# microsoft/CoCosNet

Measured on AMD Instinct MI355X. Metric: images/sec fwd+bwd ADE20k 256x256 batch-8/GPU (correspondence hot path), higher is better.
Workload: dtype f32 (K2 products as 3-term f16 hi/lo split on the f16 MFMA, fp32 accumulate); 1 GPU; ADE20k 256x256 batch 8/GPU, 64x64 grid (HW=4096), K=256, Cv=154 (rgb+151 labels), match_kernel 1, PONO_C, T=0.01; precision=f16x3; scope=hotpath: theta/phi 1x1 conv + centre/L2norm + fused corr-softmax-warp fwd+bwd; global_batch=8, parallelism=dp1, grad_payload=path, grad_allreduce_bytes=0

## Files before the change

### cocosnet_amd/csrc/corr_fused_fwd_f16x3.hip

```cpp
#include "common.h"
#include <type_traits>

namespace cocos {

typedef _Float16 f16x8 __attribute__((ext_vector_type(8)));
typedef _Float16 f16x2 __attribute__((ext_vector_type(2)));
typedef unsigned int u32x2 __attribute__((ext_vector_type(2)));

constexpr int SP_BQ = 128;
constexpr int SP_BK = 32;
constexpr int SP_KD = 256;
constexpr int SP_KROW = SP_KD + 8;
constexpr int SP_VROW = 40;
constexpr float kSplitRescaleThr = 6.0f;
constexpr float kPBias = 15.0f - kSplitRescaleThr;

__device__ __forceinline__ f32x16 mfma16h(f16x8 a, f16x8 b, f32x16 c) {
    return __builtin_amdgcn_mfma_f32_32x32x16_f16(a, b, c, 0, 0, 0);
}
__device__ __forceinline__ f16x8 buf_load_h8(__amdgpu_buffer_rsrc_t r, unsigned byte_off) {
    return __builtin_bit_cast(f16x8, __builtin_amdgcn_raw_buffer_load_b128(r, (int)byte_off, 0, 0));
}
__device__ __forceinline__ u32x4 buf_load_u4(__amdgpu_buffer_rsrc_t r, unsigned byte_off) {
    return __builtin_amdgcn_raw_buffer_load_b128(r, (int)byte_off, 0, 0);
// ... 14 lines not shown
    split_pair_rtz_lo_scaled(a, b, h, l);
    hi = __builtin_bit_cast(f16x2, h);
    lo = __builtin_bit_cast(f16x2, l);
}

constexpr int kStreamAux = 2;
#ifdef COCOS_DEBUG_TIMING
__device__ long long g_phase_fwd_h[8];
#define FPH_T(var) const long long var = __builtin_readcyclecounter()
#define FPH_ADD(i, a, b) do { if (blockIdx.x == 0 && threadIdx.x == 0) g_phase_fwd_h[i] += (b) - (a); } while (0)
#else
#define FPH_T(var) do {} while (0)
#define FPH_ADD(i, a, b) do {} while (0)
#endif

template <int CVB, bool STORE_S, bool RAGGED, bool VLO0, bool RAWM = false, int KST = SP_KD / 16>
__device__ __forceinline__ void corr_fwd_f16x3_body(
    const _Float16* __restrict__ qh, const _Float16* __restrict__ ql, const _Float16* __restrict__ kh,
    const _Float16* __restrict__ kl, const _Float16* __restrict__ vh, const _Float16* __restrict__ vl,
    float* __restrict__ out, float* __restrict__ lse, float* __restrict__ lg, const float* __restrict__ v_scale,
    const unsigned* __restrict__ v_lo_mask, int B, int Nq, int Nk, int Cv, float scale_log2 ,
    size_t k_bstride ,
    size_t v_bstride ,
    float* __restrict__ rowstat = nullptr ,
    float* __restrict__ mtile = nullptr ) {
    static_assert(KST >= 1 && KST <= SP_KD / 16 && (RAWM || KST == SP_KD / 16), "KST < 16 belongs to the magnitude-free flavour");
    constexpr int CVP = CVB * 32;
    constexpr int KPLANE = SP_BK * SP_KROW;
    constexpr int VPLANE = CVP * SP_VROW;
    extern __shared__ __attribute__((aligned(16))) unsigned char smem_raw[];
    _Float16* const kt = reinterpret_cast<_Float16*>(smem_raw);
    _Float16* const vt = kt + 2 * 2 * KPLANE;

    const int tid = threadIdx.x;
    const int lane = tid & 63, wave = tid >> 6;
    const int h = lane >> 5, c = lane & 31;

    const int nqb = (Nq + SP_BQ - 1) / SP_BQ;
    const int vb = xcd_remap(blockIdx.x, gridDim.x);
    const int b = vb / nqb, qb = vb % nqb;
    const int i_lane = qb * SP_BQ + wave * 32 + c;
// ... 123 lines not shown
    __syncthreads();

    constexpr int RA = 4, NS = SP_KD / 16;
    f16x8 ah[RA], al[RA];
    auto prefetch_k = [&](int buf) {
        const _Float16* kb = kt + buf * 2 * KPLANE + c * SP_KROW + h * 8;
#pragma unroll
        for (int s = 0; s < (RA - 1 < KST ? RA - 1 : KST); ++s) {
            ah[s] = *reinterpret_cast<const f16x8*>(kb + s * 16);
            al[s] = *reinterpret_cast<const f16x8*>(kb + KPLANE + s * 16);
        }
    };
    prefetch_k(0);

    const std::integral_constant<bool, VLO0> vlo0_tag{};
    for (int t = 0; t < ntiles; ++t) {
        const int j0 = t * SP_BK, buf = t & 1;
        const bool ragged = RAGGED && (j0 + SP_BK > Nk);
        _Float16* const kw = kt + (buf ^ 1) * 2 * KPLANE;
        _Float16* const vw = vt + (buf ^ 1) * 3 * VPLANE;
        const int jn = j0 + 2 * SP_BK;
        auto piece = [&](int i, auto vlo0_piece_tag) __attribute__((always_inline)) {
            constexpr bool PLO0 = decltype(vlo0_piece_tag)::value;
            if (!RAGGED) {
                const int jc = min(jn, Nk - SP_BK);
                if (i < 8) {
                    const int pl_ = i & 1, u = i >> 1;
                    *reinterpret_cast<u32x4*>(kw + pl_ * KPLANE + k_lds[u]) = kst[pl_][u];
                    kst[pl_][u] = buf_load_u4s(pl_ ? kl_rs : kh_rs, k_voff[u], (unsigned)jc * (unsigned)(SP_KD * 2));
                } else if (i - 8 < 2 * CVB) {
                    const int pl_ = (i - 8) & 1, u = (i - 8) >> 1;
                    if (PLO0 && pl_ == 1 && u >= 1) return;
                    const bool ones = pl_ == 0 && u == CVB - 1 && ones_thread;
                    *reinterpret_cast<u32x2*>(vw + pl_ * VPLANE + v_lds[u]) = ones ? kOnes2 : vst[pl_][u];
                    if (pl_ == 0) *reinterpret_cast<u32x2*>(vw + 2 * VPLANE + v_lds[u]) = ones ? kOnesS2 : unshift2(vst[0][u]);
                    vst[pl_][u] = buf_load_u2s(pl_ ? vl_rs : vh_rs, v_voff[u], (unsigned)jc * 2u);
                }
                return;
            }
            if (i < 8) {
                const int pl_ = i & 1, u = i >> 1;
                const int g = u * 256 + tid, key = g >> 5, cc = g & 31;
                *reinterpret_cast<u32x4*>(kw + pl_ * KPLANE + key * SP_KROW + cc * 8) = kst[pl_][u];
                kst[pl_][u] = buf_load_u4(pl_ ? kl_rs : kh_rs, (unsigned)((jn + key) * SP_KD + cc * 8) * 2u);
            } else if (i - 8 < 2 * CVB) {
                const int pl_ = (i - 8) & 1, u = (i - 8) >> 1;
                if (PLO0 && pl_ == 1 && u >= 1) return;
                const int g = u * 256 + tid, row = g >> 3, kq = g & 7;
                const int slot = 16 * (kq >> 2) + 8 * (kq & 1) + 4 * ((kq >> 1) & 1);
                const bool ones = pl_ == 0 && u == CVB - 1 && ones_thread;
                *reinterpret_cast<u32x2*>(vw + pl_ * VPLANE + row * SP_VROW + slot) = ones ? kOnes2 : vst[pl_][u];
                if (pl_ == 0) *reinterpret_cast<u32x2*>(vw + 2 * VPLANE + row * SP_VROW + slot) = ones ? kOnesS2 : unshift2(vst[0][u]);
                unsigned off = (unsigned)(row * Nk + jn + 4 * kq) * 2u;
                if (row >= Cv || jn + 4 * kq >= Nk) off = kBufOob;
                vst[pl_][u] = buf_load_u2(pl_ ? vl_rs : vh_rs, off);
            }
        };

        FPH_T(tp0);
        constexpr bool QK1 = !RAWM;
        f32x16 sa, sb, sc;
#pragma unroll
        for (int r = 0; r < 16; ++r) { sa[r] = RAWM ? -m_run : 0.f; sb[r] = RAWM ? -m_lo : 0.f; sc[r] = 0.f; }
        {
            const _Float16* kb = kt + buf * 2 * KPLANE + c * SP_KROW + h * 8;
#pragma unroll
            for (int s = 0; s < NS; ++s) {
                const int cur = s % RA;
                const bool live = s < KST;
                if (live) sa = mfma16h(ah[cur], qhr[s], sa);
                if (s + RA - 1 < KST) ah[(s + RA - 1) % RA] = *reinterpret_cast<const f16x8*>(kb + (s + RA - 1) * 16);
                __builtin_amdgcn_sched_barrier(0);
                if (live) { if (QK1) sa = mfma16h(ah[cur], qlr[s], sa); else sb = mfma16h(ah[cur], qlr[s], sb); }
                if (s + RA - 1 < KST) al[(s + RA - 1) % RA] = *reinterpret_cast<const f16x8*>(kb + KPLANE + (s + RA - 1) * 16);
                __builtin_amdgcn_sched_barrier(0);
                if (live) { if (QK1) sa = mfma16h(al[cur], qhr[s], sa); else sc = mfma16h(al[cur], qhr[s], sc); }
                if ((s & 1) == 0) piece(s >> 1, std::false_type{});
                __builtin_amdgcn_sched_barrier(0);
            }
        }
        FPH_T(tp1);
        __syncthreads();
        FPH_T(tp2);
        constexpr int NSV = 2 * CVB;
        f16x8 a_h[RA], a_l[RA], a_s[RA];
        const _Float16* vbase = vt + buf * 3 * VPLANE + c * SP_VROW + h * 8;
#pragma unroll
        for (int i = 0; i < RA - 1 && i < NSV; ++i) {
            a_h[i] = *reinterpret_cast<const f16x8*>(vbase + (i % CVB) * 32 * SP_VROW + (i / CVB) * 16);
            a_l[i] = *reinterpret_cast<const f16x8*>(vbase + VPLANE + (i % CVB) * 32 * SP_VROW + (i / CVB) * 16);
            a_s[i] = *reinterpret_cast<const f16x8*>(vbase + 2 * VPLANE + (i % CVB) * 32 * SP_VROW + (i / CVB) * 16);
        }
        f32x16 s0;
#pragma unroll
        for (int r = 0; r < 16; ++r) s0[r] = QK1 ? sa[r] : (sa[r] + sb[r]) + sc[r];
        if (ragged) {
#pragma unroll
            for (int r = 0; r < 16; ++r)
                if (j0 + acc_row_base(r) + 4 * h >= Nk) s0[r] = -INFINITY;
        }
        float tmax = s0[0];
#pragma unroll
        for (int r = 1; r < 16; ++r) tmax = fmaxf(tmax, s0[r]);
        tmax = fmaxf(tmax, swap_half(tmax));
        if (!RAWM) tmax *= scale_log2;
        if (RAWM ? (t == 0 || __any(tmax > thr_raw)) : __any(tmax > m_run + kSplitRescaleThr)) {
            float alpha;
            if (RAWM) {
                const float delta = t == 0 ? tmax : fmaxf(tmax, 0.f);
                alpha = t == 0 ? 1.0f : fast_exp2(-delta * scale_log2);
                const float u = m_lo + delta, ub = u - m_lo;
                const float e1 = (m_lo - (u - ub)) + (delta - ub);
                const float hs = m_run + u, hb = hs - m_run;
                const float e2 = (m_run - (hs - hb)) + (u - hb);
                m_run = hs;
                m_lo = e2 + e1;
#pragma unroll
                for (int r = 0; r < 16; ++r) s0[r] -= delta;
            } else {
                const float m_new = fmaxf(m_run, tmax);
                alpha = fast_exp2(m_run - m_new);
                m_run = m_new;
            }
#pragma unroll
            for (int cb = 0; cb < CVB; ++cb) asm volatile("" : "+a"(o[cb]));
#pragma unroll
            for (int cb = 0; cb < CVB; ++cb)
#pragma unroll
                for (int r = 0; r < 16; ++r) o[cb][r] *= alpha;
#pragma unroll
            for (int cb = 0; cb < CVB; ++cb) asm volatile("" : "+a"(o[cb]));
        }
        if (STORE_S) {
            const unsigned soff = (unsigned)(t * nqblk) * 4096u;
            if (RAWM && mtile && h == 0 && i_lane < Nq) {
                mtile[(((size_t)b * ntiles + t) * 2 + 0) * Nq + i_lane] = m_run;
                mtile[(((size_t)b * ntiles + t) * 2 + 1) * Nq + i_lane] = m_lo;
            }
#pragma unroll
            for (int k = 0; k < 4; ++k)
                __builtin_amdgcn_raw_buffer_store_b128(
                    __builtin_bit_cast(u32x4, f32x4{s0[4 * k], s0[4 * k + 1], s0[4 * k + 2], s0[4 * k + 3]}), lg_rs,
                    (int)lg_lane_off, (int)(soff + (unsigned)k * 1024u), kStreamAux);
        }
        float p[16];
        const float nmb = RAWM ? kPBias : kPBias - m_run;
#pragma unroll
        for (int r = 0; r < 16; ++r) p[r] = fast_exp2(__builtin_fmaf(s0[r], scale_log2, nmb));

        FPH_T(tp3);
        f16x8 ph[2], pl[2];
#pragma unroll
        for (int tt = 0; tt < 2; ++tt)
#pragma unroll
            for (int j = 0; j < 8; j += 2) {
                f16x2 a, bq;
                split_pair(p[8 * tt + j], p[8 * tt + j + 1], a, bq);
                ph[tt][j] = a[0]; ph[tt][j + 1] = a[1];
                pl[tt][j] = bq[0]; pl[tt][j + 1] = bq[1];
            }

        FPH_T(tp4);
        {
#pragma unroll
            for (int i = 0; i < NSV; ++i) {
                const int tt = i / CVB, cb = i % CVB, cur = i % RA, n = i + RA - 1;
                if (n < NSV) {
                    a_h[n % RA] = *reinterpret_cast<const f16x8*>(vbase + (n % CVB) * 32 * SP_VROW + (n / CVB) * 16);
                    a_s[n % RA] = *reinterpret_cast<const f16x8*>(vbase + 2 * VPLANE + (n % CVB) * 32 * SP_VROW + (n / CVB) * 16);
                    if (!VLO0 || (n % CVB) == 0)
                        a_l[n % RA] = *reinterpret_cast<const f16x8*>(vbase + VPLANE + (n % CVB) * 32 * SP_VROW + (n / CVB) * 16);
                }
                o[cb] = mfma16h(a_h[cur], ph[tt], o[cb]);
                o[cb] = mfma16h(a_s[cur], pl[tt], o[cb]);
                if (!VLO0 || cb == 0) o[cb] = mfma16h(a_l[cur], ph[tt], o[cb]);
                piece(8 + i, vlo0_tag);
                if (i == NSV - 1) prefetch_k(buf ^ 1);
                __builtin_amdgcn_sched_barrier(0);
            }
        }
#pragma unroll
        for (int cb = 0; cb < CVB; ++cb) asm volatile("" : "+a"(o[cb]));
        FPH_T(tp5);
        FPH_ADD(0, tp0, tp1); FPH_ADD(1, tp1, tp2); FPH_ADD(2, tp2, tp3); FPH_ADD(3, tp3, tp4);
        FPH_ADD(4, tp4, tp5);
    }

    const float l_own = o[CVB - 1][15];
    const float l_other = swap_half(l_own);
    const float l_tot = h ? l_own : l_other;
    const float inv_l = (v_scale ? 1.0f / *v_scale : 1.0f) / l_tot;
    if (RAWM && rowstat && i_lane < Nq && h == 0) {
        rowstat[((size_t)b * 3 + 0) * Nq + i_lane] = m_run;
        rowstat[((size_t)b * 3 + 1) * Nq + i_lane] = m_lo;
        rowstat[((size_t)b * 3 + 2) * Nq + i_lane] = log2f(l_tot) - kPBias;
    }
    if (RAWM) m_run = (m_run + m_lo) * scale_log2;
    if (i_lane < Nq) {
        float* out_b = out + (size_t)b * Cv * Nq;
#pragma unroll
        for (int cb = 0; cb < CVB; ++cb)
#pragma unroll
            for (int r = 0; r < 16; ++r) {
                const int ch = cb * 32 + acc_row_base(r) + 4 * h;
                if (ch < Cv) out_b[(size_t)ch * Nq + i_lane] = o[cb][r] * inv_l;
            }
        if (h == 0) lse[(size_t)b * Nq + i_lane] = (m_run + log2f(l_tot) - kPBias) * kLn2;
    }
}

template <int CVB, bool STORE_S, bool RAGGED, bool DUAL>
__global__ __launch_bounds__(256, 1) void corr_fwd_f16x3_kernel(
    const _Float16* __restrict__ qh, const _Float16* __restrict__ ql, const _Float16* __restrict__ kh,
    const _Float16* __restrict__ kl, const _Float16* __restrict__ vh, const _Float16* __restrict__ vl,
    float* __restrict__ out, float* __restrict__ lse, float* __restrict__ lg, const float* __restrict__ v_scale,
    const unsigned* __restrict__ v_lo_mask, int B, int Nq, int Nk, int Cv, float scale_log2,
    const float* __restrict__ q_scale_dev, const float* __restrict__ k_scale_dev, float* __restrict__ rowstat,
    float* __restrict__ mtile, int ksteps, size_t k_bstride, size_t v_bstride) {
    if (q_scale_dev) scale_log2 = scale_log2 / (*q_scale_dev * *k_scale_dev);
    if constexpr (DUAL) {
        if ((__builtin_amdgcn_readfirstlane(*v_lo_mask) & ~1u) == 0u)
            corr_fwd_f16x3_body<CVB, STORE_S, RAGGED, true>(qh, ql, kh, kl, vh, vl, out, lse, lg, v_scale, v_lo_mask, B, Nq, Nk, Cv, scale_log2, k_bstride, v_bstride);
        else
            corr_fwd_f16x3_body<CVB, STORE_S, RAGGED, false>(qh, ql, kh, kl, vh, vl, out, lse, lg, v_scale, v_lo_mask, B, Nq, Nk, Cv, scale_log2, k_bstride, v_bstride);
    } else {
        if (q_scale_dev) {
#define COCOS_RAWM_BODY(KST_) corr_fwd_f16x3_body<CVB, STORE_S, RAGGED, false, true, KST_>(qh, ql, kh, kl, vh, vl, out, lse, lg, v_scale, \
                                                                                           v_lo_mask, B, Nq, Nk, Cv, scale_log2, k_bstride, v_bstride, rowstat, mtile)
            if constexpr (RAGGED) {
                COCOS_RAWM_BODY(SP_KD / 16);
            } else {
                if (ksteps <= 2) COCOS_RAWM_BODY(2);
                else if (ksteps <= 4) COCOS_RAWM_BODY(4);
                else if (ksteps <= 8) COCOS_RAWM_BODY(8);
                else COCOS_RAWM_BODY(SP_KD / 16);
            }
#undef COCOS_RAWM_BODY
        } else
            corr_fwd_f16x3_body<CVB, STORE_S, RAGGED, false>(qh, ql, kh, kl, vh, vl, out, lse, lg, v_scale, v_lo_mask, B, Nq, Nk, Cv, scale_log2, k_bstride, v_bstride);
    }
}

template <int CVB, bool STORE_S, bool RAGGED, bool VLO0>
static int launch_f16x3_k(const _Float16* qh, const _Float16* ql, const _Float16* kh, const _Float16* kl,
                          const _Float16* vh, const _Float16* vl, float* out, float* lse, float* lg,
                          const float* v_scale, const unsigned* v_lo_mask, int B, int Nq, int Nk, int Cv, float scale_log2,
                          const float* qsd, const float* ksd, float* rowstat, float* mtile, int ksteps, size_t k_bstride, size_t v_bstride,
                          hipStream_t stream) {
    auto kern = corr_fwd_f16x3_kernel<CVB, STORE_S, RAGGED, VLO0>;
    const size_t smem = (size_t)2 * (2 * SP_BK * SP_KROW + 3 * CVB * 32 * SP_VROW) * sizeof(_Float16);
    COCOS_HIP_CHECK(hipFuncSetAttribute(reinterpret_cast<const void*>(kern),
                                        hipFuncAttributeMaxDynamicSharedMemorySize, (int)smem));
    const int nqb = (Nq + SP_BQ - 1) / SP_BQ;
    hipLaunchKernelGGL(kern, dim3(B * nqb), dim3(256), smem, stream, qh, ql, kh, kl, vh, vl, out, lse, lg, v_scale,
                       v_lo_mask, B, Nq, Nk, Cv, scale_log2, qsd, ksd, rowstat, mtile, ksteps, k_bstride, v_bstride);
    COCOS_HIP_CHECK(hipGetLastError());
    return COCOS_OK;
}

}

#ifdef COCOS_DEBUG_TIMING
extern "C" int cocos_debug_read_timing_fwd_f16x3(long long* host8, int reset) {
    using namespace cocos;
    COCOS_HIP_CHECK(hipDeviceSynchronize());
    COCOS_HIP_CHECK(hipMemcpyFromSymbol(host8, HIP_SYMBOL(g_phase_fwd_h), 8 * sizeof(long long)));
    if (reset) {
        long long z[8] = {0};
        COCOS_HIP_CHECK(hipMemcpyToSymbol(HIP_SYMBOL(g_phase_fwd_h), z, sizeof(z)));
    }
    return COCOS_OK;
}
#endif

template <int CVB, bool ST, bool RG, typename... A>
static int cocos_go_both(const _Float16* a, const _Float16* b2, const _Float16* c2, const _Float16* d, const _Float16* e,
                         const _Float16* f, float* out, float* lse, float* lgp, const float* v_scale_dev,
                         const unsigned* v_lo_mask_dev, A... rest) {
    using namespace cocos;
    if (CVB > 1 && v_lo_mask_dev)
        return launch_f16x3_k<CVB, ST, RG, (CVB > 1)>(a, b2, c2, d, e, f, out, lse, lgp, v_scale_dev, v_lo_mask_dev, rest...);
    return launch_f16x3_k<CVB, ST, RG, false>(a, b2, c2, d, e, f, out, lse, lgp, v_scale_dev, nullptr, rest...);
}

extern "C" size_t cocos_corr_softmax_warp_saved_logits_bytes(int B, int Nq, int Nk) {
    if (B < 1 || Nq < 1 || Nk < 1) return 0;
    return (size_t)B * ((Nk + 31) / 32) * ((Nq + 31) / 32) * 4096;
}

extern "C" int cocos_corr_softmax_warp_fwd_f16x3(const void* qh, const void* ql, const void* kh,
                                                 const void* kl, const void* vh, const void* vl, float* out,
                                                 float* lse, void* saved_logits, const float* v_scale_dev,
                                                 const unsigned* v_lo_mask_dev, int B,
                                                 int K, int Nq, int Nk, int Cv, float inv_temperature,
                                                 float operand_scale, const float* q_scale_dev, const float* k_scale_dev,
                                                 cocos_stream_t stream) {
    return cocos_corr_softmax_warp_fwd_f16x3_ex(qh, ql, kh, kl, vh, vl, out, lse, saved_logits, v_scale_dev, v_lo_mask_dev, B, K, Nq,
// ... 31 lines not shown
    COCOS_REQUIRE(!saved_logits || cocos_corr_softmax_warp_saved_logits_bytes(1, Nq, Nk) < 0x7fffffffull,
                  COCOS_ERR_UNSUPPORTED,
                  "corr_softmax_warp_fwd_f16x3: per-sample logits exceed 2 GiB; pass saved_logits = NULL");
    for (const void* p : {qh, ql, kh, kl})
        COCOS_REQUIRE(aligned16(p), COCOS_ERR_INVALID, "corr_softmax_warp_fwd_f16x3: q/k planes must be 16-byte aligned");
    for (const void* p : {vh, vl})
        COCOS_REQUIRE((reinterpret_cast<uintptr_t>(p) & 7u) == 0, COCOS_ERR_INVALID,
                      "corr_softmax_warp_fwd_f16x3: v planes must be 8-byte aligned");
    COCOS_REQUIRE(!saved_logits || aligned16(saved_logits), COCOS_ERR_INVALID,
                  "corr_softmax_warp_fwd_f16x3: saved_logits must be 16-byte aligned");
    hipStream_t s = as_stream(stream);
    COCOS_REQUIRE((q_scale_dev == nullptr) == (k_scale_dev == nullptr), COCOS_ERR_INVALID,
                  "corr_softmax_warp_fwd_f16x3: the device-side operand scales come as a pair");
    const float scale_log2 = q_scale_dev ? inv_temperature * kLog2e : inv_temperature * kLog2e / (operand_scale * operand_scale);
    const bool ragged = (Nk % SP_BK) != 0;
    const size_t k_bstride = dense_kv ? (size_t)Nk * SP_KD : 0, v_bstride = dense_kv ? (size_t)Cv * Nk : 0;
    float* lgp = static_cast<float*>(saved_logits);
    const _Float16 *a = static_cast<const _Float16*>(qh), *b2 = static_cast<const _Float16*>(ql),
                   *c2 = static_cast<const _Float16*>(kh), *d = static_cast<const _Float16*>(kl),
                   *e = static_cast<const _Float16*>(vh), *f = static_cast<const _Float16*>(vl);
#define COCOS_GO(CVB, ST, RG) \
    cocos_go_both<CVB, ST, RG>(a, b2, c2, d, e, f, out, lse, lgp, v_scale_dev, v_lo_mask_dev, B, Nq, Nk, Cv, scale_log2, \
                               q_scale_dev, k_scale_dev, rowstat_out, mtile_out, ksteps, k_bstride, v_bstride, s)
#define COCOS_CVB(CVB)                                                           \
    case CVB:                                                                    \
        if (lgp) return ragged ? COCOS_GO(CVB, true, true) : COCOS_GO(CVB, true, false); \
        return ragged ? COCOS_GO(CVB, false, true) : COCOS_GO(CVB, false, false);
    switch (Cv / 32 + 1) {
        COCOS_CVB(1) COCOS_CVB(2) COCOS_CVB(3) COCOS_CVB(4)
        default: COCOS_CVB(5)
    }
#undef COCOS_CVB
#undef COCOS_GO
}

extern "C" int cocos_corr_softmax_warp_fwd_f16x3_ex(const void* qh, const void* ql, const void* kh,
                                                    const void* kl, const void* vh, const void* vl, float* out,
                                                    float* lse, void* saved_logits, const float* v_scale_dev,
                                                    const unsigned* v_lo_mask_dev, int B,
                                                    int K, int Nq, int Nk, int Cv, float inv_temperature,
                                                    float operand_scale, const float* q_scale_dev, const float* k_scale_dev,
                                                    float* rowstat_out, float* mtile_out, int k_active, cocos_stream_t stream) {
// ... 27 lines not shown
```

### cocosnet_amd/ops.py

```python
from __future__ import annotations

import ctypes
import os
import sys
import threading
import weakref

import torch

from . import _lib

_C = _lib.CONSTANTS
CENTER_POSITIONS, CENTER_CHANNELS, CENTER_NONE = _C["COCOS_CENTER_POSITIONS"], _C["COCOS_CENTER_CHANNELS"], _C["COCOS_CENTER_NONE"]
NORM_EPS = sys.float_info.epsilon
MAX_FUSED_CV = 160
MAX_FUSED_SPLIT_CV = 159
MAX_DS_WORKSPACE_BYTES = 16 << 30
MAX_SAVED_LOGITS_BYTES = int(os.environ.get("COCOS_MAX_SAVED_LOGITS_BYTES", 16 << 30))
RECOMPUTE_CHUNK_BYTES = int(os.environ.get("COCOS_RECOMPUTE_CHUNK_BYTES", 1 << 30))
BWD_D_PRECOMPUTED = True
FUSED_K = 256
PRECISION = os.environ.get("COCOS_PRECISION", "f16x3")
PROJ_PRECISION = os.environ.get("COCOS_PROJ_PRECISION", "f16x3")
VALUE_LO_SKIP = True
PROJ_STREAM = True
SPLIT_OPERAND_SCALE = 16.0
MATCH_FUSED = True


def _stream():
    return torch.cuda.current_stream().cuda_stream


class KernelTimer:

    active = None

    def __init__(self, tags=None):
        self.events = {}
        self.tags = None if tags is None else frozenset(tags)

    def __enter__(self):
        KernelTimer.active = self
        return self

    def __exit__(self, *exc):
# ... 295 lines not shown
        ctx.split = planes is not None
        ctx.v_amax = None
        ctx.v_lomask = None
        if planes is not None:
            qh, ql, kh, kl, vh, vl, v_scale, v_amax, v_lomask = planes[:9]
            qk_scales = planes[13] if len(planes) > 13 else None
            ctx.k_active = planes[14] if len(planes) > 14 else 0
            Kp = FUSED_K if ctx.k_active else K
            ctx.recompute = bool(keep_logits) and not _saves_logits(B, Nq, Nk)
            if keep_logits and not ctx.recompute:
                nbytes = _lib.load().cocos_corr_softmax_warp_saved_logits_bytes(B, Nq, Nk)
                logits_t = torch.empty(nbytes // 4, device=qn.device, dtype=torch.float32)
            ctx.rowstat = torch.empty((B, 3, Nq), device=qn.device, dtype=torch.float32) if (qk_scales and keep_logits) else None
            ctx.mtile = (torch.empty((B, (Nk + 31) // 32, 2, Nq), device=qn.device, dtype=torch.float32)
                         if (qk_scales and logits_t is not None) else None)
            _call("corr_softmax_warp_fwd", "cocos_corr_softmax_warp_fwd_f16x3_ex", qh.data_ptr(), ql.data_ptr(),
                  kh.data_ptr(), kl.data_ptr(), vh.data_ptr(), vl.data_ptr(), out.data_ptr(), lse.data_ptr(),
                  _ptr(logits_t), v_scale.data_ptr(), _ptr(v_lomask), B, Kp, Nq, Nk, Cv, float(inv_temperature),
                  SPLIT_OPERAND_SCALE, _ptr(qk_scales[0] if qk_scales else None), _ptr(qk_scales[1] if qk_scales else None),
                  _ptr(ctx.rowstat), _ptr(ctx.mtile), ctx.k_active, _stream())
            ctx.v_amax = v_amax
            ctx.v_lomask = v_lomask
            ctx.qk_scales = qk_scales
        else:
            keep = (keep_logits and B * Nq * Nk * 4 <= MAX_DS_WORKSPACE_BYTES and Nq * Nk * 4 < 2 ** 31 - 1)
            logits_t = torch.empty((B, Nk, Nq), device=qn.device, dtype=torch.float32) if keep else None
            _call("corr_softmax_warp_fwd", "cocos_corr_softmax_warp_fwd", qn.data_ptr(), kn.data_ptr(),
                  v.data_ptr(), out.data_ptr(), lse.data_ptr(), _ptr(logits_t), B, K, Nq, Nk, Cv,
                  float(inv_temperature), _stream())
        ctx.save_for_backward(qn, kn, v, out, lse)
# ... 106 lines not shown
    kc = _recompute_chunk(B, Nq, Nk)
    ds_scale = torch.empty(1, device=dev, dtype=torch.float32)
    d_pre = _rowdot(dout, out) if BWD_D_PRECOMPUTED else None
    ka = getattr(ctx, "k_active", 0)
    Kp = FUSED_K if ka else K
    dq_acc = None
    o1 = torch.empty((B, 1, Nq), device=dev, dtype=torch.float32)
    l1 = torch.empty((B, Nq), device=dev, dtype=torch.float32)
    for k0 in range(0, Nk, kc):
        n = min(kc, Nk - k0)
        khc, klc = kh[:, k0:k0 + n].contiguous(), kl[:, k0:k0 + n].contiguous()
        vz = torch.zeros((B, 1, n), **half)
        lg = torch.empty(lib.cocos_corr_softmax_warp_saved_logits_bytes(B, Nq, n) // 4, device=dev, dtype=torch.float32)
        rowstat = getattr(ctx, "rowstat", None)
        mt = torch.empty((B, (n + 31) // 32, 2, Nq), device=dev, dtype=torch.float32) if rowstat is not None else None
        _call("corr_softmax_warp_recompute", "cocos_corr_softmax_warp_fwd_f16x3_ex", qh.data_ptr(), ql.data_ptr(), khc.data_ptr(),
              klc.data_ptr(), vz.data_ptr(), vz.data_ptr(), o1.data_ptr(), l1.data_ptr(), lg.data_ptr(), None, None, B, Kp, Nq, n, 1,
              ctx.inv_t, SPLIT_OPERAND_SCALE, _ptr(qks[0] if qks else None), _ptr(qks[1] if qks else None), None, _ptr(mt), ka, st)
        kchc, kclc = kch[:, :, k0:k0 + n].contiguous(), kcl[:, :, k0:k0 + n].contiguous()
        vphc, vplc = vph[:, k0:k0 + n].contiguous(), vpl[:, k0:k0 + n].contiguous()
        dsh = dsl = psh = psl = None
        if want_k:
            dsh, dsl = torch.empty((B, n, Nq), **half), torch.empty((B, n, Nq), **half)
        if dv is not None:
            psh, psl = torch.empty((B, n, Nq), **half), torch.empty((B, n, Nq), **half)
        blocked = int(n % 128 == 0 and Nq % 32 == 0)
        dq_c = torch.empty((B, Kp, Nq), device=dev, dtype=torch.float32)
        _call("corr_softmax_warp_bwd_query", "cocos_corr_softmax_warp_bwd_query_f16x3_ex", kchc.data_ptr(), kclc.data_ptr(),
              vphc.data_ptr(), vplc.data_ptr(), gph.data_ptr(), gpl.data_ptr(), g_scale.data_ptr(), out.data_ptr(), dout.data_ptr(),
              lse.data_ptr(), lg.data_ptr(), dq_c.data_ptr(), _ptr(dsh), _ptr(dsl), _ptr(psh), _ptr(psl), v_amax.data_ptr(),
# ... 188 lines not shown
        key = ("values", int(down), bool(patch), bool(direct_mask))
        return self._get(key, lambda: self._make["values"](int(down), bool(patch), bool(direct_mask)))


def corr_softmax_warp_shared(qh, ql, keys: PreparedKeys, values: PreparedValues, inv_temperature: float):
    B, Nq, K = qh.shape
    kh, kl, _ = keys.split_planes()
    vh, vl, v_scale, v_lomask = values.split()
    Be, Nk = kh.shape[0], kh.shape[1]
    Cv = vh.shape[1]
    if Be not in (B, 1) or vh.shape[0] != Be or vh.shape[2] != Nk or kh.shape[2] != K:
        raise ValueError(f"corr_softmax_warp_shared: shape mismatch q{tuple(qh.shape)} k{tuple(kh.shape)} v{tuple(vh.shape)}")
    dense = Be == B
    out = torch.empty((B, Cv, Nq), device=qh.device, dtype=torch.float32)
    lse = torch.empty((B, Nq), device=qh.device, dtype=torch.float32)
    _call("corr_softmax_warp_fwd", "cocos_corr_softmax_warp_fwd_f16x3_shared", qh.data_ptr(), ql.data_ptr(), kh.data_ptr(),
          kl.data_ptr(), vh.data_ptr(), vl.data_ptr(), out.data_ptr(), lse.data_ptr(), None, v_scale.data_ptr(), _ptr(v_lomask),
          B, K, Nq, Nk, Cv, float(inv_temperature), SPLIT_OPERAND_SCALE, Nk * K if dense else 0, Cv * Nk if dense else 0, _stream())
    return out


def _corr_match_planes(qh, ql, kh, kl, inv_temperature: float):
    for t in (qh, ql, kh, kl):
        if not t.is_cuda:
            raise _lib.CocosHipError("corr_match: expected CUDA/HIP operand planes; the correspondence hot path has no CPU fallback")
        if t.dtype != torch.float16 or not t.is_contiguous():
            raise TypeError("corr_match: operand planes are contiguous float16 tensors")
    B, Nq, K = qh.shape
    Be, Nk = kh.shape[0], kh.shape[1]
    if Be not in (B, 1) or kh.shape[2] != K or ql.shape != qh.shape or kl.shape != kh.shape:
# ... 2752 lines not shown
```

### include/cocos_hip.h

```cpp
#ifndef COCOS_HIP_H
#define COCOS_HIP_H

#include <stddef.h>
#include <stdint.h>

#ifdef __cplusplus
extern "C" {
#endif

#define COCOS_OK 0
#define COCOS_ERR_INVALID (-1)
#define COCOS_ERR_UNSUPPORTED (-2)
#define COCOS_ERR_HIP (-3)
#define COCOS_ERR_WORKSPACE (-4)

typedef void* cocos_stream_t;

int cocos_version(void);
const char* cocos_last_error_string(void);

#define COCOS_CENTER_POSITIONS 0
#define COCOS_CENTER_CHANNELS 1
#define COCOS_CENTER_NONE 2
int cocos_center_l2norm_fwd(const float* x, float* y, float* norm, float* row_ws,
// ... 32 lines not shown
                                      const float* q_scale_dev , const float* k_scale_dev ,
                                      cocos_stream_t stream);
int cocos_corr_softmax_warp_fwd_f16x3_ex(const void* qh, const void* ql, const void* kh, const void* kl,
                                         const void* vh, const void* vl, float* out, float* lse, void* saved_logits,
                                         const float* v_scale_dev, const unsigned* v_lo_mask_dev, int B, int K, int Nq, int Nk, int Cv,
                                         float inv_temperature, float operand_scale, const float* q_scale_dev,
                                         const float* k_scale_dev, float* rowstat_out , float* mtile_out ,
                                         int k_active ,
                                         cocos_stream_t stream);
int cocos_corr_softmax_warp_fwd_f16x3_shared(const void* qh, const void* ql, const void* kh, const void* kl,
                                             const void* vh, const void* vl, float* out, float* lse,
                                             void* saved_logits , const float* v_scale_dev,
                                             const unsigned* v_lo_mask_dev , int B, int K, int Nq, int Nk, int Cv,
                                             float inv_temperature, float operand_scale, long long k_batch_stride,
                                             long long v_batch_stride, cocos_stream_t stream);
int cocos_f16_plane_block_mask(const void* plane, int B, int C, int N, unsigned* mask_inout_dev, cocos_stream_t stream);

int cocos_split_f16_ex(const float* x, void* hi, void* lo, int B, int C, int N, int Cpad, int transpose,
                       float scale, const float* amax_dev , float* scale_out_dev ,
                       cocos_stream_t stream);
int cocos_split_f16_rows(const float* x, void* hi, void* lo, int rows, int cols, int cols_pad, float scale,
                         const float* amax_dev, float* scale_out_dev, cocos_stream_t stream);
int cocos_split_f16_transpose_pair(const float* x0, void* hi0, void* lo0, const float* amax0_dev, float* scale0_out_dev,
                                   const float* x1, void* hi1, void* lo1, const float* amax1_dev, float* scale1_out_dev, int B, int C,
                                   int N, int Cpad, cocos_stream_t stream);
int cocos_corr_softmax_warp_bwd_query_f16x3(
    const void* kch, const void* kcl, const void* vph, const void* vpl, const void* gph, const void* gpl,
    const float* g_scale_dev, const float* out, const float* dout, const float* lse, const void* saved_logits,
    float* dqn, void* dsh , void* dsl , void* psh ,
    void* psl , const float* v_amax_dev, const float* v_scale_dev ,
// ... 498 lines not shown
```

Before: 6901 images/s.

## Software-pipeline next tile's QK MFMAs under current tile's softmax in forward kernel

Adds a QK-ahead schedule to the fused f16x3 correlation forward kernel. The next key tile's QK^T MFMA chain is issued while the current tile's exp/split softmax work and first value-fragment loads are interleaved into its gaps, so MFMA and VALU work overlap instead of running serially. It applies only to the non-ragged, unit-norm flavour and is enabled by default through a new runtime switch called from Python before each forward launch. The cost is extra accumulator registers for the lookahead tile, which can lower occupancy or cause spills.

```diff
diff --git a/cocosnet_amd/csrc/corr_fused_fwd_f16x3.hip b/cocosnet_amd/csrc/corr_fused_fwd_f16x3.hip
--- a/cocosnet_amd/csrc/corr_fused_fwd_f16x3.hip
+++ b/cocosnet_amd/csrc/corr_fused_fwd_f16x3.hip
@@ -1,4 +1,5 @@
 #include "common.h"
+#include <atomic>
 #include <type_traits>
 
 namespace cocos {
@@ -52,7 +53,7 @@
 #define FPH_ADD(i, a, b) do {} while (0)
 #endif
 
-template <int CVB, bool STORE_S, bool RAGGED, bool VLO0, bool RAWM = false, int KST = SP_KD / 16>
+template <int CVB, bool STORE_S, bool RAGGED, bool VLO0, bool RAWM = false, int KST = SP_KD / 16, bool QKA = false>
 __device__ __forceinline__ void corr_fwd_f16x3_body(
     const _Float16* __restrict__ qh, const _Float16* __restrict__ ql, const _Float16* __restrict__ kh,
     const _Float16* __restrict__ kl, const _Float16* __restrict__ vh, const _Float16* __restrict__ vl,
@@ -63,6 +64,7 @@
     float* __restrict__ rowstat = nullptr ,
     float* __restrict__ mtile = nullptr ) {
     static_assert(KST >= 1 && KST <= SP_KD / 16 && (RAWM || KST == SP_KD / 16), "KST < 16 belongs to the magnitude-free flavour");
+    static_assert(!QKA || (!RAWM && !RAGGED), "the QK-ahead schedule exists for the unit-norm, whole-tile flavour only");
     constexpr int CVP = CVB * 32;
     constexpr int KPLANE = SP_BK * SP_KROW;
     constexpr int VPLANE = CVP * SP_VROW;
@@ -216,151 +218,177 @@
     prefetch_k(0);
 
     const std::integral_constant<bool, VLO0> vlo0_tag{};
-    for (int t = 0; t < ntiles; ++t) {
-        const int j0 = t * SP_BK, buf = t & 1;
-        const bool ragged = RAGGED && (j0 + SP_BK > Nk);
-        _Float16* const kw = kt + (buf ^ 1) * 2 * KPLANE;
-        _Float16* const vw = vt + (buf ^ 1) * 3 * VPLANE;
-        const int jn = j0 + 2 * SP_BK;
-        auto piece = [&](int i, auto vlo0_piece_tag) __attribute__((always_inline)) {
-            constexpr bool PLO0 = decltype(vlo0_piece_tag)::value;
-            if (!RAGGED) {
-                const int jc = min(jn, Nk - SP_BK);
-                if (i < 8) {
-                    const int pl_ = i & 1, u = i >> 1;
-                    *reinterpret_cast<u32x4*>(kw + pl_ * KPLANE + k_lds[u]) = kst[pl_][u];
-                    kst[pl_][u] = buf_load_u4s(pl_ ? kl_rs : kh_rs, k_voff[u], (unsigned)jc * (unsigned)(SP_KD * 2));
-                } else if (i - 8 < 2 * CVB) {
-                    const int pl_ = (i - 8) & 1, u = (i - 8) >> 1;
-                    if (PLO0 && pl_ == 1 && u >= 1) return;
-                    const bool ones = pl_ == 0 && u == CVB - 1 && ones_thread;
-                    *reinterpret_cast<u32x2*>(vw + pl_ * VPLANE + v_lds[u]) = ones ? kOnes2 : vst[pl_][u];
-                    if (pl_ == 0) *reinterpret_cast<u32x2*>(vw + 2 * VPLANE + v_lds[u]) = ones ? kOnesS2 : unshift2(vst[0][u]);
-                    vst[pl_][u] = buf_load_u2s(pl_ ? vl_rs : vh_rs, v_voff[u], (unsigned)jc * 2u);
-                }
-                return;
-            }
+    auto piece = [&](int i, auto vlo0_piece_tag, _Float16* const w, const int jn) __attribute__((always_inline)) {
+        constexpr bool PLO0 = decltype(vlo0_piece_tag)::value;
+        if (!RAGGED) {
+            const int jc = min(jn, Nk - SP_BK);
             if (i < 8) {
                 const int pl_ = i & 1, u = i >> 1;
-                const int g = u * 256 + tid, key = g >> 5, cc = g & 31;
-                *reinterpret_cast<u32x4*>(kw + pl_ * KPLANE + key * SP_KROW + cc * 8) = kst[pl_][u];
-                kst[pl_][u] = buf_load_u4(pl_ ? kl_rs : kh_rs, (unsigned)((jn + key) * SP_KD + cc * 8) * 2u);
+                *reinterpret_cast<u32x4*>(w + pl_ * KPLANE + k_lds[u]) = kst[pl_][u];
+                kst[pl_][u] = buf_load_u4s(pl_ ? kl_rs : kh_rs, k_voff[u], (unsigned)jc * (unsigned)(SP_KD * 2));
             } else if (i - 8 < 2 * CVB) {
                 const int pl_ = (i - 8) & 1, u = (i - 8) >> 1;
                 if (PLO0 && pl_ == 1 && u >= 1) return;
-                const int g = u * 256 + tid, row = g >> 3, kq = g & 7;
-                const int slot = 16 * (kq >> 2) + 8 * (kq & 1) + 4 * ((kq >> 1) & 1);
                 const bool ones = pl_ == 0 && u == CVB - 1 && ones_thread;
-                *reinterpret_cast<u32x2*>(vw + pl_ * VPLANE + row * SP_VROW + slot) = ones ? kOnes2 : vst[pl_][u];
-                if (pl_ == 0) *reinterpret_cast<u32x2*>(vw + 2 * VPLANE + row * SP_VROW + slot) = ones ? kOnesS2 : unshift2(vst[0][u]);
-                unsigned off = (unsigned)(row * Nk + jn + 4 * kq) * 2u;
-                if (row >= Cv || jn + 4 * kq >= Nk) off = kBufOob;
-                vst[pl_][u] = buf_load_u2(pl_ ? vl_rs : vh_rs, off);
+                *reinterpret_cast<u32x2*>(w + pl_ * VPLANE + v_lds[u]) = ones ? kOnes2 : vst[pl_][u];
+                if (pl_ == 0) *reinterpret_cast<u32x2*>(w + 2 * VPLANE + v_lds[u]) = ones ? kOnesS2 : unshift2(vst[0][u]);
+                vst[pl_][u] = buf_load_u2s(pl_ ? vl_rs : vh_rs, v_voff[u], (unsigned)jc * 2u);
             }
-        };
+            return;
+        }
+        if (i < 8) {
+            const int pl_ = i & 1, u = i >> 1;
+            const int g = u * 256 + tid, key = g >> 5, cc = g & 31;
+            *reinterpret_cast<u32x4*>(w + pl_ * KPLANE + key * SP_KROW + cc * 8) = kst[pl_][u];
+            kst[pl_][u] = buf_load_u4(pl_ ? kl_rs : kh_rs, (unsigned)((jn + key) * SP_KD + cc * 8) * 2u);
+        } else if (i - 8 < 2 * CVB) {
+            const int pl_ = (i - 8) & 1, u = (i - 8) >> 1;
+            if (PLO0 && pl_ == 1 && u >= 1) return;
+            const int g = u * 256 + tid, row = g >> 3, kq = g & 7;
+            const int slot = 16 * (kq >> 2) + 8 * (kq & 1) + 4 * ((kq >> 1) & 1);
+            const bool ones = pl_ == 0 && u == CVB - 1 && ones_thread;
+            *reinterpret_cast<u32x2*>(w + pl_ * VPLANE + row * SP_VROW + slot) = ones ? kOnes2 : vst[pl_][u];
+            if (pl_ == 0) *reinterpret_cast<u32x2*>(w + 2 * VPLANE + row * SP_VROW + slot) = ones ? kOnesS2 : unshift2(vst[0][u]);
+            unsigned off = (unsigned)(row * Nk + jn + 4 * kq) * 2u;
+            if (row >= Cv || jn + 4 * kq >= Nk) off = kBufOob;
+            vst[pl_][u] = buf_load_u2(pl_ ? vl_rs : vh_rs, off);
+        }
+    };
+
+    constexpr bool QK1 = !RAWM;
+    auto qk = [&](f32x16& sa, f32x16& sb, f32x16& sc, const int rbuf, const int jn, auto&& gap) __attribute__((always_inline)) {
+        const _Float16* kb = kt + rbuf * 2 * KPLANE + c * SP_KROW + h * 8;
+        _Float16* const kw = kt + (rbuf ^ 1) * 2 * KPLANE;
+#pragma unroll
+        for (int r = 0; r < 16; ++r) { sa[r] = RAWM ? -m_run : 0.f; sb[r] = RAWM ? -m_lo : 0.f; sc[r] = 0.f; }
+#pragma unroll
+        for (int s = 0; s < NS; ++s) {
+            const int cur = s % RA;
+            const bool live = s < KST;
+            if (live) sa = mfma16h(ah[cur], qhr[s], sa);
+            if (s + RA - 1 < KST) ah[(s + RA - 1) % RA] = *reinterpret_cast<const f16x8*>(kb + (s + RA - 1) * 16);
+            gap(3 * s);
+            __builtin_amdgcn_sched_barrier(0);
+            if (live) { if (QK1) sa = mfma16h(ah[cur], qlr[s], sa); else sb = mfma16h(ah[cur], qlr[s], sb); }
+            if (s + RA - 1 < KST) al[(s + RA - 1) % RA] = *reinterpret_cast<const f16x8*>(kb + KPLANE + (s + RA - 1) * 16);
+            gap(3 * s + 1);
+            __builtin_amdgcn_sched_barrier(0);
+            if (live) { if (QK1) sa = mfma16h(al[cur], qhr[s], sa); else sc = mfma16h(al[cur], qhr[s], sc); }
+            if ((s & 1) == 0) piece(s >> 1, std::false_type{}, kw, jn);
+            gap(3 * s + 2);
+            __builtin_amdgcn_sched_barrier(0);
+        }
+    };
+    auto no_filler = [](int) {};
+
+    f32x16 sa, sb, sc;
+    auto tile = [&](const int t, auto ahead_tag) __attribute__((always_inline)) {
+        constexpr bool AHEAD = decltype(ahead_tag)::value;
+        const int j0 = t * SP_BK, buf = t & 1;
+        const bool ragged = RAGGED && (j0 + SP_BK > Nk);
+        _Float16* const vw = vt + (buf ^ 1) * 3 * VPLANE;
+        const int jn = j0 + 2 * SP_BK;
 
         FPH_T(tp0);
-        constexpr bool QK1 = !RAWM;
-        f32x16 sa, sb, sc;
-#pragma unroll
-        for (int r = 0; r < 16; ++r) { sa[r] = RAWM ? -m_run : 0.f; sb[r] = RAWM ? -m_lo : 0.f; sc[r] = 0.f; }
-        {
-            const _Float16* kb = kt + buf * 2 * KPLANE + c * SP_KROW + h * 8;
-#pragma unroll
-            for (int s = 0; s < NS; ++s) {
-                const int cur = s % RA;
-                const bool live = s < KST;
-                if (live) sa = mfma16h(ah[cur], qhr[s], sa);
-                if (s + RA - 1 < KST) ah[(s + RA - 1) % RA] = *reinterpret_cast<const f16x8*>(kb + (s + RA - 1) * 16);
-                __builtin_amdgcn_sched_barrier(0);
-                if (live) { if (QK1) sa = mfma16h(ah[cur], qlr[s], sa); else sb = mfma16h(ah[cur], qlr[s], sb); }
-                if (s + RA - 1 < KST) al[(s + RA - 1) % RA] = *reinterpret_cast<const f16x8*>(kb + KPLANE + (s + RA - 1) * 16);
-                __builtin_amdgcn_sched_barrier(0);
-                if (live) { if (QK1) sa = mfma16h(al[cur], qhr[s], sa); else sc = mfma16h(al[cur], qhr[s], sc); }
-                if ((s & 1) == 0) piece(s >> 1, std::false_type{});
-                __builtin_amdgcn_sched_barrier(0);
-            }
-        }
+        if (!QKA) qk(sa, sb, sc, buf, jn, no_filler);
         FPH_T(tp1);
         __syncthreads();
         FPH_T(tp2);
+        if (AHEAD) prefetch_k(buf ^ 1);
         constexpr int NSV = 2 * CVB;
         f16x8 a_h[RA], a_l[RA], a_s[RA];
         const _Float16* vbase = vt + buf * 3 * VPLANE + c * SP_VROW + h * 8;
-#pragma unroll
-        for (int i = 0; i < RA - 1 && i < NSV; ++i) {
+        auto vfrag_first = [&](int i) __attribute__((always_inline)) {
+            if (i >= RA - 1 || i >= NSV) return;
             a_h[i] = *reinterpret_cast<const f16x8*>(vbase + (i % CVB) * 32 * SP_VROW + (i / CVB) * 16);
             a_l[i] = *reinterpret_cast<const f16x8*>(vbase + VPLANE + (i % CVB) * 32 * SP_VROW + (i / CVB) * 16);
             a_s[i] = *reinterpret_cast<const f16x8*>(vbase + 2 * VPLANE + (i % CVB) * 32 * SP_VROW + (i / CVB) * 16);
-        }
+        };
+        if (!AHEAD) {
+#pragma unroll
+            for (int i = 0; i < RA - 1; ++i) vfrag_first(i);
+        }
+        constexpr int NSM = 24;
         f32x16 s0;
-#pragma unroll
-        for (int r = 0; r < 16; ++r) s0[r] = QK1 ? sa[r] : (sa[r] + sb[r]) + sc[r];
-        if (ragged) {
-#pragma unroll
-            for (int r = 0; r < 16; ++r)
-                if (j0 + acc_row_base(r) + 4 * h >= Nk) s0[r] = -INFINITY;
-        }
-        float tmax = s0[0];
-#pragma unroll
-        for (int r = 1; r < 16; ++r) tmax = fmaxf(tmax, s0[r]);
-        tmax = fmaxf(tmax, swap_half(tmax));
-        if (!RAWM) tmax *= scale_log2;
-        if (RAWM ? (t == 0 || __any(tmax > thr_raw)) : __any(tmax > m_run + kSplitRescaleThr)) {
-            float alpha;
-            if (RAWM) {
-                const float delta = t == 0 ? tmax : fmaxf(tmax, 0.f);
-                alpha = t == 0 ? 1.0f : fast_exp2(-delta * scale_log2);
-                const float u = m_lo + delta, ub = u - m_lo;
-                const float e1 = (m_lo - (u - ub)) + (delta - ub);
-                const float hs = m_run + u, hb = hs - m_run;
-                const float e2 = (m_run - (hs - hb)) + (u - hb);
-                m_run = hs;
-                m_lo = e2 + e1;
-#pragma unroll
-                for (int r = 0; r < 16; ++r) s0[r] -= delta;
-            } else {
-                const float m_new = fmaxf(m_run, tmax);
-                alpha = fast_exp2(m_run - m_new);
-                m_run = m_new;
+        float p[16];
+        f16x8 ph[2], pl[2];
+        float nmb = 0.f;
+        auto sm = [&](const int g) __attribute__((always_inline)) {
+            if (g < 0) {
+#pragma unroll
+                for (int r = 0; r < 16; ++r) s0[r] = QK1 ? sa[r] : (sa[r] + sb[r]) + sc[r];
+                if (ragged) {
+#pragma unroll
+                    for (int r = 0; r < 16; ++r)
+                        if (j0 + acc_row_base(r) + 4 * h >= Nk) s0[r] = -INFINITY;
+                }
+                float tmax = s0[0];
+#pragma unroll
+                for (int r = 1; r < 16; ++r) tmax = fmaxf(tmax, s0[r]);
+                tmax = fmaxf(tmax, swap_half(tmax));
+                if (!RAWM) tmax *= scale_log2;
+                if (RAWM ? (t == 0 || __any(tmax > thr_raw)) : __any(tmax > m_run + kSplitRescaleThr)) {
+                    float alpha;
+                    if (RAWM) {
+                        const float delta = t == 0 ? tmax : fmaxf(tmax, 0.f);
+                        alpha = t == 0 ? 1.0f : fast_exp2(-delta * scale_log2);
+                        const float u = m_lo + delta, ub = u - m_lo;
+                        const float e1 = (m_lo - (u - ub)) + (delta - ub);
+                        const float hs = m_run + u, hb = hs - m_run;
+                        const float e2 = (m_run - (hs - hb)) + (u - hb);
+                        m_run = hs;
+                        m_lo = e2 + e1;
+#pragma unroll
+                        for (int r = 0; r < 16; ++r) s0[r] -= delta;
+                    } else {
+                        const float m_new = fmaxf(m_run, tmax);
+                        alpha = fast_exp2(m_run - m_new);
+                        m_run = m_new;
+                    }
+#pragma unroll
+                    for (int cb = 0; cb < CVB; ++cb) asm volatile("" : "+a"(o[cb]));
+#pragma unroll
+                    for (int cb = 0; cb < CVB; ++cb)
+#pragma unroll
+                        for (int r = 0; r < 16; ++r) o[cb][r] *= alpha;
+#pragma unroll
+                    for (int cb = 0; cb < CVB; ++cb) asm volatile("" : "+a"(o[cb]));
+                }
+                nmb = RAWM ? kPBias : kPBias - m_run;
+                return;
             }
-#pragma unroll
-            for (int cb = 0; cb < CVB; ++cb) asm volatile("" : "+a"(o[cb]));
-#pragma unroll
-            for (int cb = 0; cb < CVB; ++cb)
-#pragma unroll
-                for (int r = 0; r < 16; ++r) o[cb][r] *= alpha;
-#pragma unroll
-            for (int cb = 0; cb < CVB; ++cb) asm volatile("" : "+a"(o[cb]));
-        }
-        if (STORE_S) {
-            const unsigned soff = (unsigned)(t * nqblk) * 4096u;
-            if (RAWM && mtile && h == 0 && i_lane < Nq) {
-                mtile[(((size_t)b * ntiles + t) * 2 + 0) * Nq + i_lane] = m_run;
-                mtile[(((size_t)b * ntiles + t) * 2 + 1) * Nq + i_lane] = m_lo;
+            if (STORE_S && g < 4) {
+                const unsigned soff = (unsigned)(t * nqblk) * 4096u;
+                if (RAWM && g == 0 && mtile && h == 0 && i_lane < Nq) {
+                    mtile[(((size_t)b * ntiles + t) * 2 + 0) * Nq + i_lane] = m_run;
+                    mtile[(((size_t)b * ntiles + t) * 2 + 1) * Nq + i_lane] = m_lo;
+                }
+                __builtin_amdgcn_raw_buffer_store_b128(
+                    __builtin_bit_cast(u32x4, f32x4{s0[4 * g], s0[4 * g + 1], s0[4 * g + 2], s0[4 * g + 3]}), lg_rs,
+                    (int)lg_lane_off, (int)(soff + (unsigned)g * 1024u), kStreamAux);
             }
-#pragma unroll
-            for (int k = 0; k < 4; ++k)
-                __builtin_amdgcn_raw_buffer_store_b128(
-                    __builtin_bit_cast(u32x4, f32x4{s0[4 * k], s0[4 * k + 1], s0[4 * k + 2], s0[4 * k + 3]}), lg_rs,
-                    (int)lg_lane_off, (int)(soff + (unsigned)k * 1024u), kStreamAux);
-        }
-        float p[16];
-        const float nmb = RAWM ? kPBias : kPBias - m_run;
-#pragma unroll
-        for (int r = 0; r < 16; ++r) p[r] = fast_exp2(__builtin_fmaf(s0[r], scale_log2, nmb));
-
-        FPH_T(tp3);
-        f16x8 ph[2], pl[2];
-#pragma unroll
-        for (int tt = 0; tt < 2; ++tt)
-#pragma unroll
-            for (int j = 0; j < 8; j += 2) {
+            if (g < 16) {
+                p[g] = fast_exp2(__builtin_fmaf(s0[g], scale_log2, nmb));
+            } else if (g < NSM) {
+                const int tt = (g - 16) >> 2, j = ((g - 16) & 3) * 2;
                 f16x2 a, bq;
                 split_pair(p[8 * tt + j], p[8 * tt + j + 1], a, bq);
                 ph[tt][j] = a[0]; ph[tt][j + 1] = a[1];
                 pl[tt][j] = bq[0]; pl[tt][j + 1] = bq[1];
             }
+        };
+        sm(-1);
+        FPH_T(tp3);
+        f32x16 sn, snb, snc;
+        if (AHEAD) {
+            qk(sn, snb, snc, buf ^ 1, j0 + 3 * SP_BK, [&](const int g) __attribute__((always_inline)) {
+                if (g < NSM) sm(g);
+                if (g % 3 == 2 && g / 3 >= NS - (RA - 1)) vfrag_first(g / 3 - (NS - (RA - 1)));
+            });
+        } else {
+#pragma unroll
+            for (int g = 0; g < NSM; ++g) sm(g);
+        }
 
         FPH_T(tp4);
         {
@@ -376,8 +404,9 @@
                 o[cb] = mfma16h(a_h[cur], ph[tt], o[cb]);
                 o[cb] = mfma16h(a_s[cur], pl[tt], o[cb]);
                 if (!VLO0 || cb == 0) o[cb] = mfma16h(a_l[cur], ph[tt], o[cb]);
-                piece(8 + i, vlo0_tag);
-                if (i == NSV - 1) prefetch_k(buf ^ 1);
+                piece(8 + i, vlo0_tag, vw, jn);
+                if (!QKA && i == NSV - 1) prefetch_k(buf ^ 1);
+                if (AHEAD && i == 0) sa = sn;
                 __builtin_amdgcn_sched_barrier(0);
             }
         }
@@ -386,6 +415,13 @@
         FPH_T(tp5);
         FPH_ADD(0, tp0, tp1); FPH_ADD(1, tp1, tp2); FPH_ADD(2, tp2, tp3); FPH_ADD(3, tp3, tp4);
         FPH_ADD(4, tp4, tp5);
+    };
+    if (QKA) {
+        qk(sa, sb, sc, 0, 2 * SP_BK, no_filler);
+        for (int t = 0; t + 1 < ntiles; ++t) tile(t, std::true_type{});
+        tile(ntiles - 1, std::false_type{});
+    } else {
+        for (int t = 0; t < ntiles; ++t) tile(t, std::false_type{});
     }
 
     const float l_own = o[CVB - 1][15];
@@ -411,7 +447,7 @@
     }
 }
 
-template <int CVB, bool STORE_S, bool RAGGED, bool DUAL>
+template <int CVB, bool STORE_S, bool RAGGED, bool DUAL, bool QKA>
 __global__ __launch_bounds__(256, 1) void corr_fwd_f16x3_kernel(
     const _Float16* __restrict__ qh, const _Float16* __restrict__ ql, const _Float16* __restrict__ kh,
     const _Float16* __restrict__ kl, const _Float16* __restrict__ vh, const _Float16* __restrict__ vl,
@@ -422,9 +458,11 @@
     if (q_scale_dev) scale_log2 = scale_log2 / (*q_scale_dev * *k_scale_dev);
     if constexpr (DUAL) {
         if ((__builtin_amdgcn_readfirstlane(*v_lo_mask) & ~1u) == 0u)
-            corr_fwd_f16x3_body<CVB, STORE_S, RAGGED, true>(qh, ql, kh, kl, vh, vl, out, lse, lg, v_scale, v_lo_mask, B, Nq, Nk, Cv, scale_log2, k_bstride, v_bstride);
+            corr_fwd_f16x3_body<CVB, STORE_S, RAGGED, true, false, SP_KD / 16, QKA>(qh, ql, kh, kl, vh, vl, out, lse, lg, v_scale, v_lo_mask, B, Nq, Nk, Cv, scale_log2, k_bstride, v_bstride);
         else
-            corr_fwd_f16x3_body<CVB, STORE_S, RAGGED, false>(qh, ql, kh, kl, vh, vl, out, lse, lg, v_scale, v_lo_mask, B, Nq, Nk, Cv, scale_log2, k_bstride, v_bstride);
+            corr_fwd_f16x3_body<CVB, STORE_S, RAGGED, false, false, SP_KD / 16, QKA>(qh, ql, kh, kl, vh, vl, out, lse, lg, v_scale, v_lo_mask, B, Nq, Nk, Cv, scale_log2, k_bstride, v_bstride);
+    } else if constexpr (QKA) {
+        corr_fwd_f16x3_body<CVB, STORE_S, RAGGED, false, false, SP_KD / 16, true>(qh, ql, kh, kl, vh, vl, out, lse, lg, v_scale, v_lo_mask, B, Nq, Nk, Cv, scale_log2, k_bstride, v_bstride);
     } else {
         if (q_scale_dev) {
 #define COCOS_RAWM_BODY(KST_) corr_fwd_f16x3_body<CVB, STORE_S, RAGGED, false, true, KST_>(qh, ql, kh, kl, vh, vl, out, lse, lg, v_scale, \
@@ -443,13 +481,13 @@
     }
 }
 
-template <int CVB, bool STORE_S, bool RAGGED, bool VLO0>
+template <int CVB, bool STORE_S, bool RAGGED, bool VLO0, bool QKA>
 static int launch_f16x3_k(const _Float16* qh, const _Float16* ql, const _Float16* kh, const _Float16* kl,
                           const _Float16* vh, const _Float16* vl, float* out, float* lse, float* lg,
                           const float* v_scale, const unsigned* v_lo_mask, int B, int Nq, int Nk, int Cv, float scale_log2,
                           const float* qsd, const float* ksd, float* rowstat, float* mtile, int ksteps, size_t k_bstride, size_t v_bstride,
                           hipStream_t stream) {
-    auto kern = corr_fwd_f16x3_kernel<CVB, STORE_S, RAGGED, VLO0>;
+    auto kern = corr_fwd_f16x3_kernel<CVB, STORE_S, RAGGED, VLO0, QKA>;
     const size_t smem = (size_t)2 * (2 * SP_BK * SP_KROW + 3 * CVB * 32 * SP_VROW) * sizeof(_Float16);
     COCOS_HIP_CHECK(hipFuncSetAttribute(reinterpret_cast<const void*>(kern),
                                         hipFuncAttributeMaxDynamicSharedMemorySize, (int)smem));
@@ -475,14 +513,21 @@
 }
 #endif
 
-template <int CVB, bool ST, bool RG, typename... A>
+template <int CVB, bool ST, bool RG, bool QKA, typename... A>
 static int cocos_go_both(const _Float16* a, const _Float16* b2, const _Float16* c2, const _Float16* d, const _Float16* e,
                          const _Float16* f, float* out, float* lse, float* lgp, const float* v_scale_dev,
                          const unsigned* v_lo_mask_dev, A... rest) {
     using namespace cocos;
     if (CVB > 1 && v_lo_mask_dev)
-        return launch_f16x3_k<CVB, ST, RG, (CVB > 1)>(a, b2, c2, d, e, f, out, lse, lgp, v_scale_dev, v_lo_mask_dev, rest...);
-    return launch_f16x3_k<CVB, ST, RG, false>(a, b2, c2, d, e, f, out, lse, lgp, v_scale_dev, nullptr, rest...);
+        return launch_f16x3_k<CVB, ST, RG, (CVB > 1), QKA>(a, b2, c2, d, e, f, out, lse, lgp, v_scale_dev, v_lo_mask_dev, rest...);
+    return launch_f16x3_k<CVB, ST, RG, false, QKA>(a, b2, c2, d, e, f, out, lse, lgp, v_scale_dev, nullptr, rest...);
+}
+
+static std::atomic<int> g_fwd_qk_ahead{COCOS_FWD_QK_AHEAD_DEFAULT};
+
+extern "C" int cocos_corr_fwd_f16x3_qk_ahead(int mode) {
+    if (mode == 0 || mode == 1) return g_fwd_qk_ahead.exchange(mode, std::memory_order_relaxed);
+    return g_fwd_qk_ahead.load(std::memory_order_relaxed);
 }
 
 extern "C" size_t cocos_corr_softmax_warp_saved_logits_bytes(int B, int Nq, int Nk) {
@@ -544,18 +589,19 @@
                   "corr_softmax_warp_fwd_f16x3: the device-side operand scales come as a pair");
     const float scale_log2 = q_scale_dev ? inv_temperature * kLog2e : inv_temperature * kLog2e / (operand_scale * operand_scale);
     const bool ragged = (Nk % SP_BK) != 0;
+    const bool qka = g_fwd_qk_ahead.load(std::memory_order_relaxed) != 0 && !ragged && !q_scale_dev;
     const size_t k_bstride = dense_kv ? (size_t)Nk * SP_KD : 0, v_bstride = dense_kv ? (size_t)Cv * Nk : 0;
     float* lgp = static_cast<float*>(saved_logits);
     const _Float16 *a = static_cast<const _Float16*>(qh), *b2 = static_cast<const _Float16*>(ql),
                    *c2 = static_cast<const _Float16*>(kh), *d = static_cast<const _Float16*>(kl),
                    *e = static_cast<const _Float16*>(vh), *f = static_cast<const _Float16*>(vl);
-#define COCOS_GO(CVB, ST, RG) \
-    cocos_go_both<CVB, ST, RG>(a, b2, c2, d, e, f, out, lse, lgp, v_scale_dev, v_lo_mask_dev, B, Nq, Nk, Cv, scale_log2, \
+#define COCOS_GO(CVB, ST, RG, QKA) \
+    cocos_go_both<CVB, ST, RG, QKA>(a, b2, c2, d, e, f, out, lse, lgp, v_scale_dev, v_lo_mask_dev, B, Nq, Nk, Cv, scale_log2, \
                                q_scale_dev, k_scale_dev, rowstat_out, mtile_out, ksteps, k_bstride, v_bstride, s)
 #define COCOS_CVB(CVB)                                                           \
     case CVB:                                                                    \
-        if (lgp) return ragged ? COCOS_GO(CVB, true, true) : COCOS_GO(CVB, true, false); \
-        return ragged ? COCOS_GO(CVB, false, true) : COCOS_GO(CVB, false, false);
+        if (lgp) return ragged ? COCOS_GO(CVB, true, true, false) : qka ? COCOS_GO(CVB, true, false, true) : COCOS_GO(CVB, true, false, false); \
+        return ragged ? COCOS_GO(CVB, false, true, false) : qka ? COCOS_GO(CVB, false, false, true) : COCOS_GO(CVB, false, false, false);
     switch (Cv / 32 + 1) {
         COCOS_CVB(1) COCOS_CVB(2) COCOS_CVB(3) COCOS_CVB(4)
         default: COCOS_CVB(5)
diff --git a/cocosnet_amd/ops.py b/cocosnet_amd/ops.py
--- a/cocosnet_amd/ops.py
+++ b/cocosnet_amd/ops.py
@@ -23,6 +23,7 @@
 PRECISION = os.environ.get("COCOS_PRECISION", "f16x3")
 PROJ_PRECISION = os.environ.get("COCOS_PROJ_PRECISION", "f16x3")
 VALUE_LO_SKIP = True
+FWD_QK_AHEAD = bool(_lib.CONSTANTS["COCOS_FWD_QK_AHEAD_DEFAULT"])
 PROJ_STREAM = True
 SPLIT_OPERAND_SCALE = 16.0
 MATCH_FUSED = True
@@ -30,6 +31,10 @@
 
 def _stream():
     return torch.cuda.current_stream().cuda_stream
+
+
+def _select_fwd_schedule():
+    _lib.load().cocos_corr_fwd_f16x3_qk_ahead(1 if FWD_QK_AHEAD else 0)
 
 
 class KernelTimer:
@@ -355,6 +360,7 @@
             ctx.rowstat = torch.empty((B, 3, Nq), device=qn.device, dtype=torch.float32) if (qk_scales and keep_logits) else None
             ctx.mtile = (torch.empty((B, (Nk + 31) // 32, 2, Nq), device=qn.device, dtype=torch.float32)
                          if (qk_scales and logits_t is not None) else None)
+            _select_fwd_schedule()
             _call("corr_softmax_warp_fwd", "cocos_corr_softmax_warp_fwd_f16x3_ex", qh.data_ptr(), ql.data_ptr(),
                   kh.data_ptr(), kl.data_ptr(), vh.data_ptr(), vl.data_ptr(), out.data_ptr(), lse.data_ptr(),
                   _ptr(logits_t), v_scale.data_ptr(), _ptr(v_lomask), B, Kp, Nq, Nk, Cv, float(inv_temperature),
@@ -491,6 +497,7 @@
         lg = torch.empty(lib.cocos_corr_softmax_warp_saved_logits_bytes(B, Nq, n) // 4, device=dev, dtype=torch.float32)
         rowstat = getattr(ctx, "rowstat", None)
         mt = torch.empty((B, (n + 31) // 32, 2, Nq), device=dev, dtype=torch.float32) if rowstat is not None else None
+        _select_fwd_schedule()
         _call("corr_softmax_warp_recompute", "cocos_corr_softmax_warp_fwd_f16x3_ex", qh.data_ptr(), ql.data_ptr(), khc.data_ptr(),
               klc.data_ptr(), vz.data_ptr(), vz.data_ptr(), o1.data_ptr(), l1.data_ptr(), lg.data_ptr(), None, None, B, Kp, Nq, n, 1,
               ctx.inv_t, SPLIT_OPERAND_SCALE, _ptr(qks[0] if qks else None), _ptr(qks[1] if qks else None), None, _ptr(mt), ka, st)
@@ -709,6 +716,7 @@
     dense = Be == B
     out = torch.empty((B, Cv, Nq), device=qh.device, dtype=torch.float32)
     lse = torch.empty((B, Nq), device=qh.device, dtype=torch.float32)
+    _select_fwd_schedule()
     _call("corr_softmax_warp_fwd", "cocos_corr_softmax_warp_fwd_f16x3_shared", qh.data_ptr(), ql.data_ptr(), kh.data_ptr(),
           kl.data_ptr(), vh.data_ptr(), vl.data_ptr(), out.data_ptr(), lse.data_ptr(), None, v_scale.data_ptr(), _ptr(v_lomask),
           B, K, Nq, Nk, Cv, float(inv_temperature), SPLIT_OPERAND_SCALE, Nk * K if dense else 0, Cv * Nk if dense else 0, _stream())
diff --git a/include/cocos_hip.h b/include/cocos_hip.h
--- a/include/cocos_hip.h
+++ b/include/cocos_hip.h
@@ -70,6 +70,8 @@
                                              const unsigned* v_lo_mask_dev , int B, int K, int Nq, int Nk, int Cv,
                                              float inv_temperature, float operand_scale, long long k_batch_stride,
                                              long long v_batch_stride, cocos_stream_t stream);
+#define COCOS_FWD_QK_AHEAD_DEFAULT 1
+int cocos_corr_fwd_f16x3_qk_ahead(int mode);
 int cocos_f16_plane_block_mask(const void* plane, int B, int C, int N, unsigned* mask_inout_dev, cocos_stream_t stream);
 
 int cocos_split_f16_ex(const float* x, void* hi, void* lo, int B, int C, int N, int Cpad, int transpose,
```

New measurement: 6985 images/s (median of 6 runs). 1.2% higher.
